# apache/brpc

Hardware: NVIDIA H100
Metric: echo QPS, 1 KB baidu_std (higher is better)
Workload: dtype u8

## Files before the change

brpc_b200/csrc/b2_api.cu:

```cuda
#include <cuda_runtime.h>
#include <dlfcn.h>
#include <stdio.h>
#include <time.h>
#include <stdlib.h>
#include <string.h>
#include <mutex>
#include <string>
#include <unordered_map>
#include <vector>
#include "b2_kernels.cuh"
#include "b2_h2.cuh"

using namespace b2;

static thread_local char g_err[512] = "";
static void set_err(const char* fmt, const char* a = "", const char* b = "") { snprintf(g_err, sizeof g_err, fmt, a, b); }

#define CU(call)                                                                          \
    do {                                                                                  \
        cudaError_t e_ = (call);                                                          \
        if (e_ != cudaSuccess) { set_err("%s: %s", #call, cudaGetErrorString(e_)); return B2_E_CUDA; } \
    } while (0)

namespace {
// ... 166 lines not shown
    ALLOC(c->d_slow_idx, sizeof(uint32_t) * (size_t)o->max_msgs);
    ALLOC(c->d_heads, (size_t)kHeadBytes * (size_t)o->max_msgs);
    ALLOC(c->d_slot, 4 * ((size_t)o->max_msgs + 1));
    ALLOC(c->d_scan_tmp, 4 * (size_t)scan_blocks);
    ALLOC(c->d_resp, (size_t)c->opt.max_resp_bytes + 1024);
    ALLOC(c->d_unz, 2 * (size_t)c->opt.max_resp_bytes + 1024);
    ALLOC(c->d_snappy_tab, (size_t)kSnappyWarps * kSnappyMaxTable * 2);
    ALLOC(c->d_hpack, sizeof(HpackState) * (size_t)B2_HPACK_MAX_CONNS);
    CU(cudaMemset(c->d_hpack, 0, sizeof(HpackState) * (size_t)B2_HPACK_MAX_CONNS));
    ALLOC(c->d_counters, 8 * B2_N_COUNTERS);
    ALLOC(c->d_totals, 64);
    ALLOC(c->d_methods, sizeof(DevMethod) * 64);
    ALLOC(c->d_crc_adv, (kCrcHotWords + kCrcTreeWords) * 4);
    ALLOC(c->d_meta, (size_t)o->max_runs * 28 + 16 * (size_t)c->max_tiles + 64);
    ALLOC(c->d_small, kSmallBlock);
    HALLOC(c->h_meta, (size_t)o->max_runs * 28 + 16 * (size_t)c->max_tiles + 64);
    HALLOC(c->h_small, kSmallBlock);
    HALLOC(c->h_run_status, sizeof(b2_run_status) * (size_t)o->max_runs);
    HALLOC(c->h_msgs, sizeof(b2_msg_desc) * (size_t)o->max_msgs);
    HALLOC(c->h_refs, sizeof(b2_resp_ref) * (size_t)o->max_msgs);
    HALLOC(c->h_resp, (size_t)c->opt.max_resp_bytes);
    HALLOC(c->h_totals, 64);
    HALLOC(c->h_run_tile_base, 4 * ((size_t)o->max_runs + 1));
    CU(cudaMemset(c->d_counters, 0, 8 * B2_N_COUNTERS));
    CU(cudaMemset(c->d_bytes, 0, (size_t)o->max_batch_bytes + 1024));
    CU(cudaStreamCreateWithFlags(&c->stream, cudaStreamNonBlocking));
    for (int i = 0; i <= kMaxStages; i++) CU(cudaEventCreate(&c->ev[i]));
    CU(cudaEventCreate(&c->ev_first)); CU(cudaEventCreate(&c->ev_last));
    crc_table_init();
    CU(cudaMemcpyToSymbol(c_crc_table, g_crc_tab_host, sizeof g_crc_tab_host));
    {
        std::vector<uint32_t> tab(kCrcHotWords + kCrcTreeWords);
        auto adv = [&](uint32_t x, int bytes) { for (int k = 0; k < bytes; k++) x = g_crc_tab_host[x & 0xff] ^ (x >> 8); return x; };
        for (int k = 0; k < 16; k++) for (uint32_t b = 0; b < 256; b++) tab[k * 256 + b] = adv(g_crc_tab_host[b], k);
        for (int j = 0; j < 4; j++) for (uint32_t b = 0; b < 256; b++) tab[(16 + j) * 256 + b] = adv(b << (8 * j), 512);
        for (int t = 0; t < 5; t++) for (int j = 0; j < 4; j++) for (uint32_t b = 0; b < 256; b++)
            tab[kCrcHotWords + (t * 4 + j) * 256 + b] = adv(b << (8 * j), 16 << t);
        CU(cudaMemcpy(c->d_crc_adv, tab.data(), tab.size() * 4, cudaMemcpyHostToDevice));
    }
    CU(cudaFuncSetAttribute(k_resolve, cudaFuncAttributeMaxDynamicSharedMemorySize, 200 * 1024));
    CU(cudaFuncSetAttribute(k_pack_slow<false>, cudaFuncAttributeMaxDynamicSharedMemorySize, (int)(8 * kSnapRing)));
    CU(cudaFuncSetAttribute(k_pack_tma<kPackGroup>, cudaFuncAttributeMaxDynamicSharedMemorySize, (int)(sizeof(PackWarpSmem) * kPackWarps)));
    CU(cudaFuncSetAttribute(k_pack_tma<kPackGroupSmall>, cudaFuncAttributeMaxDynamicSharedMemorySize, (int)(sizeof(PackWarpSmem) * kPackWarps)));
    if (const char* e = getenv("B2_PACK")) c->use_tma_pack = strcmp(e, "reg") != 0;
    if (const char* e = getenv("B2_SMALL")) c->use_fused_small = strcmp(e, "off") != 0;
    if (const char* e = getenv("B2_FUSED")) c->use_fused = strcmp(e, "off") != 0;
    CU(cudaFuncSetAttribute(k_fused, cudaFuncAttributeMaxDynamicSharedMemorySize, (int)(sizeof(FusedWarpSmem) * (kFusedWarps > kFusedWarpsDense ? kFusedWarps : kFusedWarpsDense))));
    CU(cudaFuncSetAttribute(k_small, cudaFuncAttributeMaxDynamicSharedMemorySize, (int)sizeof(SmallSmem)));
    *out = c;
    return B2_OK;
}

extern "C" int b2_set_server_identity(b2_ctx* c, const char* ip_port) {
    if (!c) return B2_E_INVAL;
    const size_t n = ip_port ? strlen(ip_port) : 0;
    if (n >= sizeof c->cfg.identity) { set_err("identity too long"); return B2_E_INVAL; }
    memset(c->cfg.identity, 0, sizeof c->cfg.identity);
    if (n) memcpy(c->cfg.identity, ip_port, n);
    c->cfg.identity_len = (uint32_t)n;
    return B2_OK;
}

extern "C" int b2_set_modes(b2_ctx* c, int input_mode, int resp_mode) {
    if (!c || (input_mode != B2_INPUT_COPY && input_mode != B2_INPUT_PULL) || (resp_mode != B2_RESP_COPY && resp_mode != B2_RESP_BY_REF && resp_mode != B2_RESP_IOVEC)) { set_err("bad mode"); return B2_E_INVAL; }
    static_assert(sizeof(b2_resp_ref) == sizeof(uint4), "b2_resp_ref is 16 bytes");
    static_assert(sizeof(b2_iovec) == sizeof(ulonglong2) && sizeof(void*) == 8, "b2_iovec is a 16-byte struct iovec");
    if (resp_mode == B2_RESP_IOVEC && !c->d_iov) {
        CU(cudaSetDevice(c->opt.device));
        if (cudaMalloc((void**)&c->d_iov, 32 * (size_t)c->opt.max_msgs) != cudaSuccess || cudaHostAlloc((void**)&c->h_iov, 32 * (size_t)c->opt.max_msgs, cudaHostAllocDefault) != cudaSuccess) {
            cudaFree(c->d_iov); c->d_iov = nullptr; cudaGetLastError(); set_err("allocation of the iovec list failed"); return B2_E_NOMEM;
        }
    }
    if (input_mode == B2_INPUT_PULL && !c->d_rows) {
        CU(cudaSetDevice(c->opt.device));
        const uint32_t tile = c->adaptive_tile ? 32768u : c->opt.tile_bytes;
        const size_t tiles = (size_t)c->opt.max_batch_bytes / tile + c->opt.max_runs + 1;
        const size_t rows = tiles * (tile >= 2048 ? kSpecKDense : kSpecK);
        if (cudaMalloc((void**)&c->d_rows, rows * 128) != cudaSuccess || cudaMalloc((void**)&c->d_frame_row, 4 * (size_t)c->opt.max_msgs) != cudaSuccess) {
            cudaFree(c->d_rows); c->d_rows = nullptr; cudaGetLastError(); set_err("cudaMalloc of the pull-mode row stash failed"); return B2_E_NOMEM;
        }
    }
    ring_halt(c);
    c->input_mode = input_mode; c->resp_mode = resp_mode; c->cfg.by_ref = resp_mode != B2_RESP_COPY; c->cfg.pull = input_mode == B2_INPUT_PULL; c->cfg.pull_vecs = resp_mode != B2_RESP_COPY ? 6u : 8u;
    c->uploaded = false; c->executed = false;
    return B2_OK;
}

extern "C" int b2_set_protocols(b2_ctx* c, uint32_t mask) {
    const uint32_t known = (1u << 1) | (1u << 2) | (1u << 3) | (1u << 4) | (1u << 12);
    if (!c || mask == 0 || (mask & ~known)) { set_err("unknown protocol in mask (baidu_std 1, streaming_rpc 2, hulu_pbrpc 3, sofa_pbrpc 4, nshead 12)"); return B2_E_INVAL; }
    ring_halt(c);
    c->cfg.proto_mask = mask;
    return B2_OK;
}

extern "C" int b2_set_stream_handler(b2_ctx* c, int kind) {
    if (!c || (kind != B2_STREAM_DESC_ONLY && kind != B2_STREAM_SNAPPY_UNCOMPRESS)) { set_err("bad stream handler"); return B2_E_INVAL; }
    c->cfg.stream_handler = (uint32_t)kind;
    return B2_OK;
}

extern "C" int b2_register_method(b2_ctx* c, const b2_method* m) {
    if (!c || !m || !m->service_full_name || !m->service_name || !m->method_name || !m->request_type_name) { set_err("null argument"); return B2_E_INVAL; }
    if (c->methods.size() >= 64) { set_err("method table full"); return B2_E_CAPACITY; }
    DevMethod d; memset(&d, 0, sizeof d);
    std::string full = std::string(m->service_full_name) + "." + m->method_name;
    if (full.size() >= sizeof d.full_method || strlen(m->service_name) >= sizeof d.service_short ||
        strlen(m->service_full_name) >= sizeof d.service_full || strlen(m->request_type_name) >= sizeof d.request_type) {
        set_err("method names too long"); return B2_E_INVAL;
    }
    memcpy(d.full_method, full.data(), full.size()); d.full_method_len = (uint32_t)full.size();
    d.service_short_len = (uint32_t)strlen(m->service_name); memcpy(d.service_short, m->service_name, d.service_short_len);
    d.service_full_len = (uint32_t)strlen(m->service_full_name); memcpy(d.service_full, m->service_full_name, d.service_full_len);
    d.request_type_len = (uint32_t)strlen(m->request_type_name); memcpy(d.request_type, m->request_type_name, d.request_type_len);
    d.handler = m->handler; d.echo_attachment = m->echo_attachment;
    d.response_checksum_type = m->response_checksum_type; d.response_compress_type = m->response_compress_type;
    ring_halt(c);
    c->methods.push_back(d);
    c->cfg.n_methods = (uint32_t)c->methods.size();
    CU(cudaSetDevice(c->opt.device));
    CU(cudaMemcpy(c->d_methods, c->methods.data(), sizeof(DevMethod) * c->methods.size(), cudaMemcpyHostToDevice));
    return (int)c->methods.size() - 1;
}

static BatchPtrs make_ptrs(b2_ctx* c) {
    BatchPtrs B;
    B.bytes = c->d_bytes; B.runs = c->d_runs; B.run_tile_base = c->d_run_tile_base; B.tiles = c->d_tiles;
    B.tile_base = c->d_tile_base; B.tile_scratch = c->d_tile_scratch; B.tile_spec = c->d_tile_spec; B.run_status = c->d_run_status; B.frame_off = c->d_frame_off; B.frame_run = c->d_frame_run; B.frame_row = c->d_frame_row; B.rows = c->d_rows; B.msgs = c->d_msgs;
    B.aux = c->d_aux; B.jobs = c->d_jobs; B.refs = c->d_refs; B.slow_idx = c->d_slow_idx; B.heads = c->d_heads; B.slot = c->d_slot; B.scan_tmp = c->d_scan_tmp; B.resp = c->d_resp; B.unz = c->d_unz; B.snappy_tab = c->d_snappy_tab; B.counters = c->d_counters;
    B.totals = c->d_totals; B.methods = c->d_methods; B.crc_adv = c->d_crc_adv;
    B.n_runs = c->n_runs; B.n_tiles = c->n_tiles; B.max_msgs = c->opt.max_msgs; B.max_resp = c->opt.max_resp_bytes;
    B.runs = reinterpret_cast<const b2_run*>(c->d_meta);
    B.run_tile_base = reinterpret_cast<const uint32_t*>(c->d_meta + (size_t)c->n_runs * sizeof(b2_run));
    B.tile_info = reinterpret_cast<const uint4*>(c->d_meta + c->meta_tile_off);
    if (c->input_mode == B2_INPUT_PULL) B.bytes = c->pull_bytes;
    if (c->small) {
        B.refs = reinterpret_cast<uint4*>(c->d_small + c->small_off_refs);
        B.totals = reinterpret_cast<uint32_t*>(c->d_small);
        B.run_status = reinterpret_cast<b2_run_status*>(c->d_small + c->small_off_rs);
        B.msgs = reinterpret_cast<b2_msg_desc*>(c->d_small + c->small_off_msgs);
        B.resp = c->d_small + c->small_off_resp;
        B.max_msgs = c->small_msgs; B.max_resp = c->small_resp;
    }
    return B;
}

extern "C" int b2_batch_upload(b2_ctx* c, const void* bytes, uint32_t nbytes, const b2_run* runs, uint32_t n_runs) {
    if (!c || (!bytes && nbytes) || (!runs && n_runs)) { set_err("null argument"); return B2_E_INVAL; }
    if ((c->input_mode != B2_INPUT_PULL && nbytes > c->opt.max_batch_bytes) || nbytes >= (1u << 31) || n_runs > c->opt.max_runs) { set_err("batch exceeds ctx capacity"); return B2_E_CAPACITY; }
    uint64_t covered = 0; for (uint32_t r = 0; r < n_runs; r++) covered += runs[r].length;
    if (c->input_mode == B2_INPUT_PULL && covered > c->opt.max_batch_bytes) { set_err("runs exceed ctx capacity"); return B2_E_CAPACITY; }
    c->covered = covered;
    CU(cudaSetDevice(c->opt.device));
    if (c->adaptive_tile) {
        uint32_t t = 8192;
        const uint32_t per_tile = c->input_mode == B2_INPUT_PULL ? 48u : 6u;
        if (c->input_mode == B2_INPUT_PULL && t < 32768) t = 32768;
        while (t < (1u << 20) && t < per_tile * c->avg_frame) t <<= 1;
        c->cfg.tile_bytes = t; c->cfg.tile_shift = 0; while ((1u << c->cfg.tile_shift) < t) c->cfg.tile_shift++;
    }
    const uint32_t shift = c->cfg.tile_shift, tile = c->cfg.tile_bytes;
    c->dense = tile >= 2048 && c->avg_frame && (uint64_t)c->avg_frame * kSpecK < tile;
    c->cfg.spec_k = c->dense ? kSpecKDense : kSpecK;
    uint64_t nt = 0; uint32_t max_rt = 0;
    for (uint32_t r = 0; r < n_runs; r++) {
        if ((runs[r].offset & 15u) || (uint64_t)runs[r].offset + runs[r].length > nbytes) { set_err("run offset must be 16-aligned and inside the batch"); return B2_E_INVAL; }
        c->h_run_tile_base[r] = (uint32_t)nt;
        const uint32_t t = (uint32_t)(((uint64_t)runs[r].length + tile - 1) >> shift);
        nt += t; if (t > max_rt) max_rt = t;
    }
    c->h_run_tile_base[n_runs] = (uint32_t)nt;
    if (nt > c->max_tiles) { set_err("too many tiles"); return B2_E_CAPACITY; }
    c->n_runs = n_runs; c->n_tiles = (uint32_t)nt; c->nbytes = nbytes; c->max_run_tiles = max_rt; c->host_bytes = bytes;
    const size_t tile_off = ((size_t)n_runs * sizeof(b2_run) + 4 * ((size_t)n_runs + 1) + 15) & ~(size_t)15;
    const size_t meta_bytes = tile_off + 16 * (size_t)nt;
    c->meta_tile_off = tile_off;
    if (n_runs) memcpy(c->h_meta, runs, (size_t)n_runs * sizeof(b2_run));
    memcpy(c->h_meta + (size_t)n_runs * sizeof(b2_run), c->h_run_tile_base, 4 * ((size_t)n_runs + 1));
    {
        uint32_t* ti = reinterpret_cast<uint32_t*>(c->h_meta + tile_off);
        for (uint32_t r = 0; r < n_runs; r++) {
            const uint32_t t0 = c->h_run_tile_base[r], t1 = c->h_run_tile_base[r + 1];
            for (uint32_t t = t0; t < t1; t++) { uint32_t* q = ti + 4 * (size_t)t; q[0] = runs[r].offset; q[1] = runs[r].length; q[2] = t - t0; q[3] = r | (runs[r].flags << 24); }
        }
    }
    c->h2_last_in = 0; c->h2_last_out = 0;
    if (c->input_mode == B2_INPUT_PULL) {
        void* dp = nullptr;
        if (nbytes && cudaHostGetDevicePointer(&dp, const_cast<void*>(bytes), 0) != cudaSuccess) {
            cudaGetLastError(); set_err("B2_INPUT_PULL: bytes must be pinned + mapped memory from b2_block_alloc"); return B2_E_INVAL;
        }
        c->pull_bytes = static_cast<const uint8_t*>(dp);
    } else if (nbytes) CU(cudaMemcpyAsync(c->d_bytes, bytes, nbytes, cudaMemcpyHostToDevice, c->stream));
    CU(cudaMemcpyAsync(c->d_meta, c->h_meta, meta_bytes, cudaMemcpyHostToDevice, c->stream));
    c->small = c->allow_small && nbytes <= kSmallBytes && n_runs <= kSmallRuns && n_runs > 0;
    if (c->small) {
        uint32_t mb = nbytes / 12 + 1; if (mb > kSmallMsgs) mb = kSmallMsgs;
        if (mb > c->opt.max_msgs) mb = c->opt.max_msgs;
        c->small_msgs = mb; c->small_resp = nbytes + mb * 80 + 2048;
        c->small_off_rs = 64; c->small_off_msgs = 64 + n_runs * 32; c->small_off_refs = c->small_off_msgs + mb * 64;
        c->small_off_resp = (c->small_off_refs + mb * 16 + 255u) & ~255u;
        c->small_total = c->small_off_resp + c->small_resp;
    }
    if (const char* e = getenv("B2_STAGE_MASK")) c->stage_mask = (uint32_t)atoi(e);
    c->uploaded = true; c->executed = false;
    return B2_OK;
}

static int launch_pipeline(b2_ctx* c) {
    const BatchPtrs B = make_ptrs(c);
    DevConfig C = c->cfg;
    const bool fused = c->use_fused && !c->slow_heavy && !c->small && c->input_mode == B2_INPUT_COPY && c->resp_mode == B2_RESP_COPY && c->use_tma_pack &&
                       (((uint64_t)c->nbytes + 255) & ~255ull) + 4096 <= c->opt.max_resp_bytes;
    C.fused = fused ? 1u : 0u; C.ovf_base = (c->nbytes + 255u) & ~255u; c->fused_last = fused;
    cudaStream_t s = c->stream;
    int st = 0; uint32_t launches = 0;
    const bool prof = c->profile_stages;
    auto mark = [&](const char* name) { if (prof) { c->stage_names[st] = name; cudaEventRecord(c->ev[st + 1], s); st++; } };
    const uint32_t mask = c->stage_mask;
    if (mask & 1) CU(cudaMemsetAsync(B.totals, 0, 48, s));
    CU(cudaEventRecord(c->ev[0], s));
    if (c->n_runs == 0) { c->n_stages = 0; c->last_launches = 0; return B2_OK; }
    if (c->small && c->use_fused_small && !prof) {
        k_small<<<1, kSmallThreads, sizeof(SmallSmem), s>>>(B, C);
        c->stage_names[0] = "fused_small"; cudaEventRecord(c->ev[1], s);
        c->n_stages = 1; c->last_launches = 1;
        CU(cudaGetLastError());
        return B2_OK;
    }
    const uint32_t sms = c->n_sms;
    if (mask & 1) {
    if (c->n_tiles) {
        k_tile_search<<<(c->n_tiles * 32 + 255) / 256, 256, 0, s>>>(B, C); launches++; mark("tile_search");
        if (C.pull) k_tile_walk_pull<<<(uint32_t)(((uint64_t)c->n_tiles * 8 + 127) / 128), 128, 0, s>>>(B, C);
        else k_tile_walk<<<(c->n_tiles + 127) / 128, 128, 0, s>>>(B, C);
        launches++; mark("tile_walk");
    }
    {
        size_t smem = (size_t)c->max_run_tiles * 12;
        if (smem > 200 * 1024) smem = 0;
        k_resolve<<<c->n_runs, 256, smem, s>>>(B, C, smem == 0 ? 1u : 0u); launches++; mark("resolve");
    }
    if (fused) {
        const uint32_t fw = c->avg_frame && !c->dense ? kFusedWarps : kFusedWarpsDense;
        if (c->n_tiles) { k_fused<<<sms, fw * 32, sizeof(FusedWarpSmem) * fw, s>>>(B, C); launches++; mark("fused"); }
    } else {
    if (c->n_tiles) { k_frame_table<<<(uint32_t)(((uint64_t)c->n_tiles * C.spec_k + 255) / 256), 256, 0, s>>>(B, C); launches++; mark("frame_table"); }
    k_decode<<<sms * B2_DECODE_MIN_BLOCKS, kDecodeWarps * 32, 0, s>>>(B, C); launches++; mark("decode");
    k_scan_blocks<<<sms, kScanBlock, 0, s>>>(B); launches++;
    mark("scan");
    }
    }
    if (fused) {
        if (mask & 4) { k_pack_slow<true><<<sms * B2_SLOW_MIN_BLOCKS, 256, 0, s>>>(B, C); launches++; mark("pack_slow"); }
    } else if (c->use_tma_pack) {
        if (mask & 4) {
            if (c->slow_heavy || c->cfg.by_ref) { C.verify_done = 1; k_crc_verify<<<sms * 6, 256, 0, s>>>(B, C); launches++; mark("crc_verify"); }
            k_pack_slow<false><<<sms * B2_SLOW_MIN_BLOCKS, 256, 8 * kSnapRing, s>>>(B, C); launches++; mark("pack_slow");
        }
        if (mask & 2) {
            if ((c->avg_frame && c->avg_frame < 640) || c->cfg.by_ref) k_pack_tma<kPackGroupSmall><<<sms, kPackWarps * 32, sizeof(PackWarpSmem) * kPackWarps, s>>>(B, C);
            else k_pack_tma<kPackGroup><<<sms, kPackWarps * 32, sizeof(PackWarpSmem) * kPackWarps, s>>>(B, C);
            launches++; mark("pack");
        }
    } else { k_pack<<<sms * B2_PACK_MIN_BLOCKS, 256, 0, s>>>(B, C); launches++; mark("pack"); }
    if (c->resp_mode == B2_RESP_IOVEC && !c->small) {
        k_emit_iov<<<sms * 4, 256, 0, s>>>(B, c->d_iov, (unsigned long long)(uintptr_t)c->h_resp, (unsigned long long)(uintptr_t)c->host_bytes);
        launches++; mark("emit_iov");
    }
    if (!prof) { c->stage_names[0] = "pipeline"; cudaEventRecord(c->ev[1], s); st = 1; }
    c->n_stages = st; c->last_launches = launches;
    CU(cudaGetLastError());
    return B2_OK;
}

extern "C" int b2_batch_execute(b2_ctx* c, float* kernel_ms, uint32_t* n_launches) {
    if (!c || !c->uploaded) { set_err("no batch uploaded"); return B2_E_INVAL; }
    CU(cudaSetDevice(c->opt.device));
    c->profile_stages = true;
    int rc = launch_pipeline(c);
    c->profile_stages = false;
    if (rc != B2_OK) return rc;
    CU(cudaStreamSynchronize(c->stream));
    float ms = 0.f;
    if (c->n_stages) CU(cudaEventElapsedTime(&ms, c->ev[0], c->ev[c->n_stages]));
    c->last_kernel_ms = ms; c->executed = true;
    if (kernel_ms) *kernel_ms = ms;
    if (n_launches) *n_launches = c->last_launches;
    return B2_OK;
}

extern "C" int b2_batch_execute_many(b2_ctx* c, uint32_t steps, float* total_ms, uint32_t* n_launches) {
    if (!c || !c->uploaded || steps == 0) { set_err("no batch uploaded"); return B2_E_INVAL; }
    CU(cudaSetDevice(c->opt.device));
    cudaEvent_t e0, e1;
    CU(cudaEventCreate(&e0)); CU(cudaEventCreate(&e1));
    CU(cudaEventRecord(e0, c->stream));
    uint32_t launches = 0;
    for (uint32_t i = 0; i < steps; i++) {
        int rc = launch_pipeline(c);
        if (rc != B2_OK) return rc;
        launches += c->last_launches;
    }
    CU(cudaEventRecord(e1, c->stream));
    CU(cudaStreamSynchronize(c->stream));
    float ms = 0.f;
    CU(cudaEventElapsedTime(&ms, e0, e1));
    cudaEventDestroy(e0); cudaEventDestroy(e1);
    c->executed = true;
    if (c->n_stages) { float t = 0.f; cudaEventElapsedTime(&t, c->ev[0], c->ev[c->n_stages]); c->last_kernel_ms = t; }
    if (total_ms) *total_ms = ms;
    if (n_launches) *n_launches = launches;
    return B2_OK;
}

extern "C" int b2_batch_launch(b2_ctx* c) {
    if (!c || !c->uploaded) { set_err("no batch uploaded"); return B2_E_INVAL; }
    CU(cudaSetDevice(c->opt.device));
    if (c->first_pending) { CU(cudaEventRecord(c->ev_first, c->stream)); c->first_pending = false; }
    int rc = launch_pipeline(c);
    if (rc != B2_OK) return rc;
    CU(cudaEventRecord(c->ev_last, c->stream));
    c->executed = true;
    return B2_OK;
}
extern "C" int b2_batch_wait(b2_ctx* c) {
    if (!c) return B2_E_INVAL;
    CU(cudaSetDevice(c->opt.device));
    CU(cudaStreamSynchronize(c->stream));
    c->first_pending = true;
    return B2_OK;
}
extern "C" int b2_elapsed_ms(b2_ctx* a, b2_ctx* b, float* ms) {
    if (!a || !b || !ms) return B2_E_INVAL;
    CU(cudaSetDevice(a->opt.device));
    CU(cudaEventElapsedTime(ms, a->ev_first, b->ev_last));
    return B2_OK;
}

static void refs_to_iov(b2_ctx* c, b2_batch_result* out, const void* host_bytes) {
    b2_run_status* rs = const_cast<b2_run_status*>(out->runs);
    for (uint32_t r = 0; r < out->n_runs; r++) rs[r].n_unanswered = 0;
    for (uint32_t i = 0; i < out->n_msgs; i++) {
        const b2_msg_desc& d = out->msgs[i];
        b2_iovec a = { const_cast<uint8_t*>(out->resp), 0 }, b = a;
        if (d.status == B2_MSG_ECHOED || d.status == B2_MSG_ERROR_REPLIED) {
            const b2_resp_ref rf = d.status == B2_MSG_ECHOED ? out->refs[i] : b2_resp_ref{0, 0, 0, 0};
            a.iov_base = const_cast<uint8_t*>(out->resp) + d.resp_off; a.iov_len = rf.src_len ? rf.prefix_len : d.resp_len;
            if (rf.src_len) { b.iov_base = const_cast<uint8_t*>(static_cast<const uint8_t*>(host_bytes)) + rf.src_off; b.iov_len = rf.src_len; }
        } else rs[d.run_idx].n_unanswered++;
        c->h_iov[2 * (size_t)i] = a; c->h_iov[2 * (size_t)i + 1] = b;
    }
    out->iov = c->h_iov; out->refs = nullptr;
}

static int download_normal(b2_ctx* c, b2_batch_result* out) {
    CU(cudaMemcpyAsync(c->h_totals, c->d_totals, 48, cudaMemcpyDeviceToHost, c->stream));
    CU(cudaStreamSynchronize(c->stream));
    if (c->n_runs && c->fused_last) {
        const bool heavy = (uint64_t)c->h_totals[3] * 8 > c->h_totals[0];
        if ((c->h_totals[2] & 2u) && !(c->h_totals[2] & 1u)) {
            c->slow_heavy = true;
            int rc = launch_pipeline(c); if (rc != B2_OK) return rc;
            CU(cudaMemcpyAsync(c->h_totals, c->d_totals, 48, cudaMemcpyDeviceToHost, c->stream));
            CU(cudaStreamSynchronize(c->stream));
        }
        c->slow_heavy = heavy || c->slow_heavy;
    } else if (c->n_runs && c->slow_heavy && !c->small) {
        c->slow_heavy = ((uint64_t)c->h_totals[3] + c->h_totals[7]) * 8 > c->h_totals[0];
    }
    if (c->n_runs && (c->h_totals[2] & 3u)) {
        set_err(c->h_totals[2] & 1u ? "more messages than max_msgs" : "responses exceed max_resp_bytes"); return B2_E_CAPACITY;
    }
    if (c->n_runs && c->fused_last) c->h_totals[1] = ((c->nbytes + 255u) & ~255u) + c->h_totals[9];
    const uint32_t n_msgs = c->n_runs ? c->h_totals[0] : 0, resp_bytes = c->n_runs ? c->h_totals[1] : 0;
    if (c->n_runs) CU(cudaMemcpyAsync(c->h_run_status, c->d_run_status, sizeof(b2_run_status) * c->n_runs, cudaMemcpyDeviceToHost, c->stream));
    if (n_msgs) CU(cudaMemcpyAsync(c->h_msgs, c->d_msgs, sizeof(b2_msg_desc) * (size_t)n_msgs, cudaMemcpyDeviceToHost, c->stream));
    if (resp_bytes) CU(cudaMemcpyAsync(c->h_resp, c->d_resp, resp_bytes, cudaMemcpyDeviceToHost, c->stream));
    const bool iovec = c->resp_mode == B2_RESP_IOVEC;
    if (n_msgs && c->cfg.by_ref && !iovec) CU(cudaMemcpyAsync(c->h_refs, c->d_refs, sizeof(b2_resp_ref) * (size_t)n_msgs, cudaMemcpyDeviceToHost, c->stream));
    if (n_msgs && iovec) CU(cudaMemcpyAsync(c->h_iov, c->d_iov, 32 * (size_t)n_msgs, cudaMemcpyDeviceToHost, c->stream));
    CU(cudaStreamSynchronize(c->stream));
    out->refs = c->cfg.by_ref && !iovec ? c->h_refs : nullptr;
    out->iov = iovec ? c->h_iov : nullptr;
    out->runs = c->h_run_status; out->n_runs = c->n_runs;
    out->msgs = c->h_msgs; out->n_msgs = n_msgs;
    out->resp = c->h_resp; out->resp_bytes = resp_bytes;
    return B2_OK;
}

extern "C" int b2_batch_download(b2_ctx* c, b2_batch_result* out) {
    if (!c || !out || !c->executed) { set_err("no executed batch"); return B2_E_INVAL; }
    CU(cudaSetDevice(c->opt.device));
    memset(out, 0, sizeof *out);
    if (c->small) {
        if (!c->small_copy_queued) CU(cudaMemcpyAsync(c->h_small, c->d_small, c->small_total, cudaMemcpyDeviceToHost, c->stream));
        c->small_copy_queued = false;
        CU(cudaStreamSynchronize(c->stream));
        const uint32_t* tot = reinterpret_cast<const uint32_t*>(c->h_small);
        if (tot[2] & 3u) {
            c->small = false;
            int rc = launch_pipeline(c);
            if (rc != B2_OK) return rc;
            rc = download_normal(c, out);
            if (rc != B2_OK) return rc;
        } else {
            out->runs = reinterpret_cast<const b2_run_status*>(c->h_small + c->small_off_rs); out->n_runs = c->n_runs;
// ... 798 lines not shown
```

brpc_b200/csrc/b2_kernels.cuh:

```cuda
#pragma once
#include <cuda_runtime.h>
#include "b2_core.cuh"
#include "b2_inflate.cuh"

namespace b2 {

enum TileKind : uint8_t { kRanOff = 0, kStop = 1, kAmbig = 2 };

struct __align__(16) TileRec {
    uint32_t entry;
    uint32_t exit;
    uint32_t count;
    uint8_t kind;
    int8_t last_proto;
    uint8_t live;
    int8_t pf_in;
};

struct __align__(16) MsgAux {
    uint32_t msg_off;
    uint32_t msg_len;
    uint32_t att_len;
    uint32_t att_off;
    uint32_t cks_off;
    uint32_t cks_len;
    uint32_t svc_off, svc_len;
    uint32_t mth_off, mth_len;
    uint32_t pad;
    uint32_t err_kind;
};
struct __align__(16) PackJob {
    uint32_t src_off;
    uint32_t bulk_len;
    uint16_t head_len;
    uint8_t pad;
    uint8_t fast;
    uint32_t slot_len;
};
constexpr uint32_t kHeadBytes = 96;

enum ErrKind : uint32_t { kErrNone = 0, kErrAttachment, kErrNoService, kErrNoMethod, kErrParseRequest };

struct DevMethod {
    char full_method[200];
    uint32_t full_method_len;
    char service_short[64];  uint32_t service_short_len;
    char service_full[120];  uint32_t service_full_len;
    char request_type[96];   uint32_t request_type_len;
    int32_t handler, echo_attachment, response_checksum_type, response_compress_type;
};
struct DevConfig {
    uint64_t max_body_size;
    uint32_t tile_bytes, tile_shift;
    uint32_t n_methods;
    uint32_t identity_len;
    uint32_t stream_handler;
    uint32_t spec_k;
    uint32_t by_ref;
    uint32_t verify_done;
    uint32_t proto_mask;
    uint32_t fused;
    uint32_t ovf_base;
    uint32_t pull_vecs;
    uint32_t pull;
    char identity[64];
};

struct BatchPtrs {
    const uint8_t* bytes;
    const b2_run* runs;
    const uint32_t* run_tile_base;
    const uint4* tile_info;
    TileRec* tiles;
    uint32_t* tile_base;
    uint32_t* tile_scratch;
    uint32_t* tile_spec;
    b2_run_status* run_status;
    uint32_t* frame_off;
    uint32_t* frame_run;
    uint32_t* frame_row;
    uint4* rows;
    b2_msg_desc* msgs;
    MsgAux* aux;
    PackJob* jobs;
    uint4* refs;
    uint32_t* slow_idx;
    uint8_t* heads;
    uint32_t* slot;
    uint32_t* scan_tmp;
    uint8_t* resp;
    uint8_t* unz;
    uint16_t* snappy_tab;
    unsigned long long* counters;
    uint32_t* totals;
    const DevMethod* methods;
    const uint32_t* crc_adv;
    uint32_t n_runs, n_tiles, max_msgs, max_resp;
};

template <bool kSpec, typename Emit>
B2_HD void walk_tile(const uint8_t* run, uint32_t len, uint32_t entry, int pf_in, uint32_t tile_end,
                     uint64_t max_body, bool client, TileRec& t, Emit emit, uint32_t mask = kProtoMaskDefault) {
    uint32_t pos = entry, count = 0;
    int pf = kSpec ? -1 : pf_in, last = 0;
    uint8_t kind = kRanOff;
    while (pos < tile_end) {
        const Step s = cut_input_message(run, len, pos, pf, max_body, client, mask);
        if (kSpec && count == 0 && (s.popped || (s.index != 12 && nshead_claims(run, len, pos, max_body, mask)))) { kind = kAmbig; break; }
        if (s.err != B2_PARSE_OK) { kind = kStop; break; }
        emit(count, s);
        count++; last = s.index; pf = s.index; pos = s.new_pos;
    }
    t.entry = entry; t.exit = pos; t.count = count; t.kind = kind; t.last_proto = (int8_t)last;
}
struct NoEmit { B2_HD void operator()(uint32_t, const Step&) const {} };
constexpr uint32_t kSpecK = 16;
constexpr uint32_t kSpecKDense = 128;
constexpr uint8_t kKindRewalked = 0x80;
struct EmitSpec {
    uint32_t* out; uint32_t run_off, cap;
    __device__ __forceinline__ void operator()(uint32_t i, const Step& s) const {
        if (i < cap) out[i] = (run_off + s.frame_pos) | ((uint32_t)(s.index != 1) << 31);
    }
};

#if defined(__CUDACC__)

__device__ __forceinline__ uint32_t find_run(const uint32_t* base, uint32_t n_runs, uint32_t tile) {
    uint32_t lo = 0, hi = n_runs;
    while (hi - lo > 1) { const uint32_t mid = (lo + hi) >> 1; if (__ldg(base + mid) <= tile) lo = mid; else hi = mid; }
    return lo;
}
__device__ __forceinline__ bool is_magic(uint32_t w) { return w == kMagicPRPC || w == kMagicSTRM; }
#ifndef B2_SEARCH_FIRST
#define B2_SEARCH_FIRST 2
#endif

__global__ void __launch_bounds__(256, 6) k_tile_search(BatchPtrs B, DevConfig C) {
    const uint32_t warp = (blockIdx.x * blockDim.x + threadIdx.x) >> 5, lane = threadIdx.x & 31;
    if (warp >= B.n_tiles) return;
    const uint4 ti = __ldg(B.tile_info + warp);
    const uint32_t k = ti.z;
    const uint8_t* base = B.bytes + ti.x;
    const uint32_t len = ti.y;
    uint32_t entry = kNone;
    if (k == 0) {
        entry = 0;
    } else {
        const uint32_t t0 = k << C.tile_shift;
        const uint32_t t1 = min(t0 + C.tile_bytes, len);
        for (uint32_t c0 = t0; c0 < t1 && entry == kNone; c0 += (c0 == t0 ? 512u * B2_SEARCH_FIRST : 2048u)) {
            const int nwin = c0 == t0 ? B2_SEARCH_FIRST : 4;
            uint4 v[4]; uint32_t nx[4];
            #pragma unroll
            for (int u = 0; u < 4; u++) {
                const uint32_t p0 = c0 + u * 512 + lane * 16;
                v[u] = make_uint4(0, 0, 0, 0); nx[u] = 0;
                if (u < nwin && p0 < t1) {
                    v[u] = __ldg(reinterpret_cast<const uint4*>(base + p0));
                    nx[u] = __ldg(reinterpret_cast<const uint32_t*>(base + p0 + 16));
                }
            }
            #pragma unroll
            for (int u = 0; u < 4; u++) {
                if (entry != kNone || u >= nwin) break;
                const uint32_t w0 = c0 + u * 512, p0 = w0 + lane * 16;
                const uint32_t w[5] = { v[u].x, v[u].y, v[u].z, v[u].w, nx[u] };
                uint32_t mask = 0, mkind = 0;
                const bool ext = (C.proto_mask & ((1u << 3) | (1u << 4))) != 0;
                #pragma unroll
                for (int k4 = 0; k4 < 4; k4++) {
                    uint32_t e = __vcmpeq4(w[k4], 0x50505050u) | __vcmpeq4(w[k4], 0x53535353u);
                    if (ext) e |= __vcmpeq4(w[k4], 0x48484848u);
                    while (e) {
                        const int b = (__ffs(e) - 1) >> 3;
                        e &= ~(0xffu << (8 * b));
                        const int j = 4 * k4 + b;
                        const uint32_t word = __funnelshift_r(w[k4], w[k4 + 1], b * 8);
                        const bool other = ext && ((word == kMagicHULU && (C.proto_mask & 8u)) || (word == kMagicSOFA && (C.proto_mask & 16u)));
                        if ((is_magic(word) || other) && p0 + j + 4 <= len && p0 + j < t1) { mask |= 1u << j; if (other) mkind |= (word == kMagicHULU ? 1u : 2u) << (2 * j); }
                    }
                }
                uint32_t any = __ballot_sync(0xffffffffu, mask != 0);
                const uint32_t n5 = __shfl_down_sync(0xffffffffu, v[u].y, 1), n6 = __shfl_down_sync(0xffffffffu, v[u].z, 1);
                while (any && entry == kNone) {
                    const int src = __ffs(any) - 1;
                    uint32_t m = __shfl_sync(0xffffffffu, mask, src);
                    const uint32_t kinds = __shfl_sync(0xffffffffu, mkind, src);
                    while (m && entry == kNone) {
                        const int jj = __ffs(m) - 1;
                        const uint32_t p = w0 + src * 16 + jj;
                        m &= m - 1;
                        const uint32_t kind = (kinds >> (2 * jj)) & 3u;
                        if (kind == 2) { entry = p; break; }
                        uint32_t body_le = 0, meta_le = 0;
                        if (src < 31) {
                            const uint32_t q = (uint32_t)(jj + 4) >> 2, sh = ((uint32_t)(jj + 4) & 3u) * 8u;
                            const uint32_t a1 = w[1], a2 = w[2], a3 = w[3], a4 = w[4];
                            const uint32_t x0 = q == 1 ? a1 : q == 2 ? a2 : q == 3 ? a3 : a4;
                            const uint32_t x1 = q == 1 ? a2 : q == 2 ? a3 : q == 3 ? a4 : n5;
                            const uint32_t x2 = q == 1 ? a3 : q == 2 ? a4 : q == 3 ? n5 : n6;
                            body_le = __shfl_sync(0xffffffffu, __funnelshift_r(x0, x1, sh), src);
                            meta_le = __shfl_sync(0xffffffffu, __funnelshift_r(x1, x2, sh), src);
                        } else if (p + 12 <= len) {
                            body_le = load_le32(base + p + 4); meta_le = load_le32(base + p + 8);
                        } else continue;
                        const uint32_t body = kind == 1 ? body_le : __byte_perm(body_le, 0, 0x0123), meta = kind == 1 ? meta_le : __byte_perm(meta_le, 0, 0x0123);
                        if (meta <= body && (uint64_t)body <= C.max_body_size) entry = p;
                    }
                    any &= any - 1;
                }
            }
        }
    }
    if (lane == 0) B.tiles[warp].entry = entry;
}

struct HdrWords { uint32_t w0, w1, w2, w3; };
__device__ __forceinline__ HdrWords load_hdr_words(const uint8_t* p) {
    const uint32_t* q = reinterpret_cast<const uint32_t*>((uintptr_t)p & ~(uintptr_t)3);
    HdrWords h; h.w0 = __ldg(q); h.w1 = __ldg(q + 1); h.w2 = __ldg(q + 2); h.w3 = __ldg(q + 3);
    return h;
}
template <typename Emit>
__device__ __forceinline__ void walk_tile_spec(const uint8_t* run, uint32_t len, uint32_t entry, uint32_t tile_end,
                                               uint64_t max_body, bool client, TileRec& t, Emit emit, uint32_t mask) {
    uint32_t pos = entry, count = 0, prev_len = 0, pre_pos = kNone;
    int pf = -1, last = 0;
    uint8_t kind = kRanOff;
    HdrWords pre; pre.w0 = pre.w1 = pre.w2 = pre.w3 = 0;
    while (pos < tile_end) {
        Step s;
        bool fast = false;
        if (len - pos >= 12) {
            const HdrWords h = pre_pos == pos ? pre : load_hdr_words(run + pos);
            const uint32_t guess = pos + prev_len;
            if (prev_len && guess < tile_end && (uint64_t)guess + 12 <= len) { pre = load_hdr_words(run + guess); pre_pos = guess; }
            else pre_pos = kNone;
            const uint32_t sh = 8u * (pos & 3u);
            const uint32_t h0 = sh ? __funnelshift_r(h.w0, h.w1, sh) : h.w0, h1 = sh ? __funnelshift_r(h.w1, h.w2, sh) : h.w1,
                           h2 = sh ? __funnelshift_r(h.w2, h.w3, sh) : h.w2;
            const int idx = h0 == kMagicPRPC ? 1 : h0 == kMagicSTRM ? 2 : 0;
            const uint32_t body = __byte_perm(h1, 0, 0x0123), meta = __byte_perm(h2, 0, 0x0123);
            if (idx && ((mask >> idx) & 1u) && pf != 12 && (uint64_t)body <= max_body && (uint64_t)(len - pos) >= 12ull + body && meta <= body) {
                s.err = B2_PARSE_OK; s.index = idx; s.pf = idx; s.frame_pos = pos; s.new_pos = pos + 12 + body; s.body = body; s.meta = meta; s.popped = false;
                fast = true;
            }
        }
        if (!fast) s = cut_input_message(run, len, pos, pf, max_body, client, mask);
        if (count == 0 && (s.popped || (s.index != 12 && nshead_claims(run, len, pos, max_body, mask)))) { kind = kAmbig; break; }
        if (s.err != B2_PARSE_OK) { kind = kStop; break; }
        emit(count, s);
        count++; last = s.index; pf = s.index; prev_len = s.new_pos - pos; pos = s.new_pos;
    }
    t.entry = entry; t.exit = pos; t.count = count; t.kind = kind; t.last_proto = (int8_t)last;
}

__global__ void __launch_bounds__(128) k_tile_walk(BatchPtrs B, DevConfig C) {
    const uint32_t t = blockIdx.x * blockDim.x + threadIdx.x;
    if (t >= B.n_tiles) return;
    const uint4 ti = __ldg(B.tile_info + t);
    const uint32_t k = ti.z;
    b2_run run; run.offset = ti.x; run.length = ti.y; run.flags = ti.w >> 24;
    TileRec rec;
    rec.entry = B.tiles[t].entry; rec.exit = 0; rec.count = 0; rec.kind = kStop; rec.last_proto = 0; rec.live = 0; rec.pf_in = -1;
    if (rec.entry != kNone) {
        EmitSpec e; e.out = B.tile_spec + (size_t)t * C.spec_k; e.run_off = run.offset; e.cap = C.spec_k;
        walk_tile_spec(B.bytes + run.offset, run.length, rec.entry, (k + 1) << C.tile_shift, C.max_body_size, (run.flags & B2_RUN_CLIENT) != 0, rec, e, run_mask(C.proto_mask, run.flags));
    }
    B.tiles[t] = rec;
}

__global__ void __launch_bounds__(128) k_tile_walk_pull(BatchPtrs B, DevConfig C) {
    const uint32_t g = blockIdx.x * blockDim.x + threadIdx.x;
    const uint32_t t = g >> 3, sub = threadIdx.x & 7u, lane = threadIdx.x & 31u;
    if (t >= B.n_tiles) return;
    const uint32_t gmask = 0xffu << (lane & 24u), l0 = lane & 24u;
    const uint4 ti = __ldg(B.tile_info + t);
    const uint32_t k = ti.z, len = ti.y;
    const uint8_t* run = B.bytes + ti.x;
    const bool client = ((ti.w >> 24) & B2_RUN_CLIENT) != 0;
    const uint32_t pmask = run_mask(C.proto_mask, ti.w >> 24);
    const uint32_t tile_end = (k + 1) << C.tile_shift, cap = C.spec_k;
    uint32_t* spec = B.tile_spec + (size_t)t * cap;
    uint4* rows = B.rows + (size_t)t * cap * 8;
    TileRec rec;
    rec.entry = B.tiles[t].entry; rec.exit = 0; rec.count = 0; rec.kind = kStop; rec.last_proto = 0; rec.live = 0; rec.pf_in = -1;
    if (rec.entry != kNone) {
        uint32_t pos = rec.entry, count = 0; int pf = -1, last = 0; uint8_t kind = kRanOff;
        while (pos < tile_end) {
            bool fast = false; uint32_t new_pos = pos, frame_pos = pos; int idx = 0, err = B2_PARSE_OK; bool popped = false;
            uint4 v = make_uint4(0, 0, 0, 0);
            if (len - pos >= 12) {
                if (sub < C.pull_vecs) v = __ldg(reinterpret_cast<const uint4*>(run + (pos & ~15u)) + sub);
                const uint32_t a0 = __shfl_sync(gmask, v.x, l0), a1 = __shfl_sync(gmask, v.y, l0), a2 = __shfl_sync(gmask, v.z, l0), a3 = __shfl_sync(gmask, v.w, l0);
                const uint32_t b0 = __shfl_sync(gmask, v.x, l0 + 1), b1 = __shfl_sync(gmask, v.y, l0 + 1), b2 = __shfl_sync(gmask, v.z, l0 + 1);
                const uint32_t q = (pos & 15u) >> 2, sh = 8u * (pos & 3u);
                const uint32_t w0 = q == 0 ? a0 : q == 1 ? a1 : q == 2 ? a2 : a3, w1 = q == 0 ? a1 : q == 1 ? a2 : q == 2 ? a3 : b0;
                const uint32_t w2 = q == 0 ? a2 : q == 1 ? a3 : q == 2 ? b0 : b1, w3 = q == 0 ? a3 : q == 1 ? b0 : q == 2 ? b1 : b2;
                const uint32_t h0 = sh ? __funnelshift_r(w0, w1, sh) : w0, h1 = sh ? __funnelshift_r(w1, w2, sh) : w1, h2 = sh ? __funnelshift_r(w2, w3, sh) : w2;
                idx = h0 == kMagicPRPC ? 1 : h0 == kMagicSTRM ? 2 : 0;
                const uint32_t body = __byte_perm(h1, 0, 0x0123), meta = __byte_perm(h2, 0, 0x0123);
                if (idx && ((pmask >> idx) & 1u) && pf != 12 && (uint64_t)body <= C.max_body_size && (uint64_t)(len - pos) >= 12ull + body && meta <= body) { fast = true; new_pos = pos + 12 + body; }
            }
            if (count == 0 && ((pmask >> 12) & 1u)) {
                int amb = 0;
                if (sub == 0) amb = nshead_claims(run, len, pos, C.max_body_size, pmask) ? 1 : 0;
                if (__shfl_sync(gmask, amb, l0)) { kind = kAmbig; break; }
            }
            if (!fast) {
                Step s; s.err = 0; s.index = 0; s.new_pos = 0; s.frame_pos = 0; s.popped = false;
                if (sub == 0) s = cut_input_message(run, len, pos, pf, C.max_body_size, client, pmask);
                err = __shfl_sync(gmask, s.err, l0); idx = __shfl_sync(gmask, s.index, l0); new_pos = __shfl_sync(gmask, s.new_pos, l0);
                frame_pos = __shfl_sync(gmask, s.frame_pos, l0); popped = __shfl_sync(gmask, (int)s.popped, l0) != 0;
                if (count == 0 && popped) { kind = kAmbig; break; }
                if (err != B2_PARSE_OK) { kind = kStop; break; }
                if (sub < C.pull_vecs) v = __ldg(reinterpret_cast<const uint4*>(run + (frame_pos & ~15u)) + sub);
            }
            if (count < cap) {
                if (sub == 0) spec[count] = (ti.x + frame_pos) | ((uint32_t)(idx != 1) << 31);
                if (sub < C.pull_vecs) rows[(size_t)count * 8 + sub] = v;
            }
            count++; last = idx; pf = idx; pos = new_pos;
        }
        rec.exit = pos; rec.count = count; rec.kind = kind; rec.last_proto = (int8_t)last;
    }
    if (sub == 0) B.tiles[t] = rec;
}

__device__ __forceinline__ void run_prefix_body(const BatchPtrs& B, uint32_t* s_warp, uint32_t* s_carry) {
    const uint32_t lane = threadIdx.x & 31, wid = threadIdx.x >> 5, nw = blockDim.x >> 5;
    if (threadIdx.x == 0) *s_carry = 0;
    __syncthreads();
    for (uint32_t base = 0; base < B.n_runs; base += blockDim.x) {
        const uint32_t i = base + threadIdx.x;
        uint32_t v = i < B.n_runs ? __ldcg(&B.run_status[i].n_msgs) : 0, x = v;
        #pragma unroll
        for (int d = 1; d < 32; d <<= 1) { const uint32_t y = __shfl_up_sync(0xffffffffu, x, d); if (lane >= (uint32_t)d) x += y; }
        if (lane == 31) s_warp[wid] = x;
        __syncthreads();
        uint32_t wbase = 0, wtot = 0;
        for (uint32_t w = 0; w < nw; w++) { const uint32_t t = s_warp[w]; if (w < wid) wbase += t; wtot += t; }
        const uint32_t carry = *s_carry;
        if (i < B.n_runs) B.run_status[i].first_msg = carry + wbase + x - v;
        __syncthreads();
        if (threadIdx.x == 0) *s_carry = carry + wtot;
        __syncthreads();
    }
    if (threadIdx.x == 0) { B.totals[0] = *s_carry; if (*s_carry > B.max_msgs) B.totals[2] |= 1u; }
}

constexpr uint32_t kLinkOk = 0x80000000u;
constexpr uint32_t kLinkStop = 0x40000000u;
constexpr uint32_t kLinkEnd = 0x20000000u;
constexpr uint32_t kLinkBroken = 0x10000000u;
constexpr uint32_t kLinkRewalk = 0x08000000u;

__device__ __forceinline__ uint32_t make_link(const TileRec& t, const TileRec* tiles, uint32_t nt, uint32_t shift) {
    if (t.entry == kNone || t.kind == kAmbig) return kLinkRewalk;
    if (t.kind == kStop) return kLinkStop;
    const uint32_t j = t.exit >> shift;
    if (j >= nt) return kLinkEnd;
    return (tiles[j].entry == t.exit ? kLinkOk : kLinkBroken) | j;
}

__global__ void __launch_bounds__(256) k_resolve(BatchPtrs B, DevConfig C, uint32_t use_scratch) {
    extern __shared__ uint32_t sm[];
    const uint32_t r = blockIdx.x;
    const b2_run run = B.runs[r];
    const uint8_t* base = B.bytes + run.offset;
    const uint32_t len = run.length;
    const uint32_t tb = B.run_tile_base[r], nt = B.run_tile_base[r + 1] - tb;
    TileRec* tiles = B.tiles + tb;
    const bool fits = !use_scratch;
    uint32_t* link = fits ? sm : B.tile_scratch + 3ull * tb;
    uint32_t* cp = link + nt;
    uint32_t* live = cp + nt;
    __shared__ uint32_t s_final_pos, s_warp_sum[8], s_warp_pf[8], s_carry_sum, s_carry_pf;
    const uint32_t rmask = run_mask(C.proto_mask, run.flags);
    const bool pf_decides = (run.flags & B2_RUN_CLIENT) && !(rmask & kProtoMaskDump) && (rmask & ~((1u << B2_PROTOCOL_BAIDU_STD) | (1u << B2_PROTOCOL_STREAMING_RPC))) != 0;
    for (uint32_t k = threadIdx.x; k < nt; k += blockDim.x) {
        const TileRec t = tiles[k];
        link[k] = ((k == 0 && t.entry != 0) || pf_decides) ? kLinkRewalk : make_link(t, tiles, nt, C.tile_shift);
        cp[k] = (t.count << 4) | ((uint32_t)t.last_proto & 15u);
        live[k] = 0;
    }
    __shared__ uint32_t s_first_bad;
    if (threadIdx.x == 0) s_first_bad = nt ? nt - 1 : 0;
    __syncthreads();
    {
        uint32_t mine = nt;
        for (uint32_t k = threadIdx.x; k + 1 < nt; k += blockDim.x)
            if (link[k] != (kLinkOk | (k + 1))) { mine = k; break; }
        if (mine < nt) atomicMin(&s_first_bad, mine);
    }
    __syncthreads();
    const uint32_t first_bad = s_first_bad;
    for (uint32_t k = threadIdx.x; k < first_bad; k += blockDim.x) live[k] = 1;
    __syncthreads();
    if (threadIdx.x == 0) {
        uint32_t k = first_bad, pos = 0;
        bool via_ok = first_bad > 0;
        while (k < nt) {
            uint32_t v = link[k];
            if (v & kLinkRewalk) {
                if (via_ok) pos = tiles[k].entry;
                int pf = run.preferred_proto;
                for (uint32_t j = k; j-- > 0;) if (live[j] && (cp[j] >> 4)) { pf = (int)(cp[j] & 15u); break; }
                TileRec t; t.live = 0; t.pf_in = 0;
                walk_tile<false>(base, len, pos, pf, (k + 1) << C.tile_shift, C.max_body_size, (run.flags & B2_RUN_CLIENT) != 0, t, NoEmit(), run_mask(C.proto_mask, run.flags));
                tiles[k].entry = t.entry; tiles[k].exit = t.exit; tiles[k].count = t.count; tiles[k].kind = t.kind | kKindRewalked; tiles[k].last_proto = t.last_proto;
                cp[k] = (t.count << 4) | ((uint32_t)t.last_proto & 15u);
                v = make_link(t, tiles, nt, C.tile_shift);
                link[k] = v;
            }
            live[k] = 1;
            if (v & kLinkOk) { k = v & 0x07ffffffu; via_ok = true; continue; }
            if (v & kLinkBroken) {
                const uint32_t j = v & 0x07ffffffu;
                pos = tiles[k].exit; k = j; link[j] = kLinkRewalk; via_ok = false;
                continue;
            }
            pos = tiles[k].exit;
// ... 2120 lines not shown
```

Before: 1.020 billion.

## Fuse tile search and walk into persistent speculative-stride front kernel

For non-pull input, tile entry search and the tile walk are merged into one persistent kernel, k_tile_front, which takes work chunks through an atomic counter. Each 8-lane group walks its tile speculatively at a predicted frame stride and validates several candidate headers in parallel. It falls back to the serial parser when the guess fails, and issues L2 prefetches for the search region. The change also seeds avg_frame on the host from the first frame header of each run, and relaunches pack_slow with twice the blocks at 128 threads each. The goal is fewer launches and less serial per-frame walking, at the cost of more divergence and complexity. It also depends on a counter slot (totals+10) that is zeroed by the existing memset.

Measured after the change: 1.094 billion (median of 6 runs). +7.2%, better.

```diff
diff --git a/brpc_b200/csrc/b2_api.cu b/brpc_b200/csrc/b2_api.cu
--- a/brpc_b200/csrc/b2_api.cu
+++ b/brpc_b200/csrc/b2_api.cu
@@ -342,6 +342,16 @@
     if (c->input_mode == B2_INPUT_PULL && covered > c->opt.max_batch_bytes) { set_err("runs exceed ctx capacity"); return B2_E_CAPACITY; }
     c->covered = covered;
     CU(cudaSetDevice(c->opt.device));
+    if (!c->avg_frame && n_runs) {
+        uint64_t sum = 0; uint32_t n = 0;
+        for (uint32_t r = 0; r < n_runs; r++) {
+            if (runs[r].length < 12 || (uint64_t)runs[r].offset + 12 > nbytes) continue;
+            const uint8_t* p = static_cast<const uint8_t*>(bytes) + runs[r].offset;
+            const uint32_t magic = load_le32(p), body = load_be32(p + 4);
+            if ((magic == kMagicPRPC || magic == kMagicSTRM) && body <= c->cfg.max_body_size) { sum += 12ull + body; n++; }
+        }
+        if (n) c->avg_frame = (uint32_t)(sum / n);
+    }
     if (c->adaptive_tile) {
         uint32_t t = 8192;
         const uint32_t per_tile = c->input_mode == B2_INPUT_PULL ? 48u : 6u;
@@ -420,11 +430,12 @@
     }
     const uint32_t sms = c->n_sms;
     if (mask & 1) {
-    if (c->n_tiles) {
+    if (c->n_tiles && C.pull) {
         k_tile_search<<<(c->n_tiles * 32 + 255) / 256, 256, 0, s>>>(B, C); launches++; mark("tile_search");
-        if (C.pull) k_tile_walk_pull<<<(uint32_t)(((uint64_t)c->n_tiles * 8 + 127) / 128), 128, 0, s>>>(B, C);
-        else k_tile_walk<<<(c->n_tiles + 127) / 128, 128, 0, s>>>(B, C);
-        launches++; mark("tile_walk");
+        k_tile_walk_pull<<<(uint32_t)(((uint64_t)c->n_tiles * 8 + 127) / 128), 128, 0, s>>>(B, C); launches++; mark("tile_walk");
+    } else if (c->n_tiles) {
+        const uint32_t chunks = (c->n_tiles + 8 * kFrontChunk - 1) / (8 * kFrontChunk), grid = chunks < sms * 4 ? chunks : sms * 4;
+        k_tile_front<<<grid, 256, 0, s>>>(B, C); launches++; mark("tile_front");
     }
     {
         size_t smem = (size_t)c->max_run_tiles * 12;
@@ -442,7 +453,7 @@
     }
     }
     if (fused) {
-        if (mask & 4) { k_pack_slow<true><<<sms * B2_SLOW_MIN_BLOCKS, 256, 0, s>>>(B, C); launches++; mark("pack_slow"); }
+        if (mask & 4) { k_pack_slow<true><<<sms * B2_SLOW_MIN_BLOCKS * 2, 128, 0, s>>>(B, C); launches++; mark("pack_slow"); }
     } else if (c->use_tma_pack) {
         if (mask & 4) {
             if (c->slow_heavy || c->cfg.by_ref) { C.verify_done = 1; k_crc_verify<<<sms * 6, 256, 0, s>>>(B, C); launches++; mark("crc_verify"); }
diff --git a/brpc_b200/csrc/b2_kernels.cuh b/brpc_b200/csrc/b2_kernels.cuh
--- a/brpc_b200/csrc/b2_kernels.cuh
+++ b/brpc_b200/csrc/b2_kernels.cuh
@@ -136,14 +136,10 @@
 #define B2_SEARCH_FIRST 2
 #endif
 
-__global__ void __launch_bounds__(256, 6) k_tile_search(BatchPtrs B, DevConfig C) {
-    const uint32_t warp = (blockIdx.x * blockDim.x + threadIdx.x) >> 5, lane = threadIdx.x & 31;
-    if (warp >= B.n_tiles) return;
-    const uint4 ti = __ldg(B.tile_info + warp);
-    const uint32_t k = ti.z;
-    const uint8_t* base = B.bytes + ti.x;
-    const uint32_t len = ti.y;
+__device__ __forceinline__ uint32_t search_tile_entry(const uint8_t* base, uint32_t len, uint32_t k, uint32_t lane, const DevConfig& C,
+                                                      uint32_t& first_len) {
     uint32_t entry = kNone;
+    first_len = 0;
     if (k == 0) {
         entry = 0;
     } else {
@@ -206,13 +202,22 @@
                             body_le = load_le32(base + p + 4); meta_le = load_le32(base + p + 8);
                         } else continue;
                         const uint32_t body = kind == 1 ? body_le : __byte_perm(body_le, 0, 0x0123), meta = kind == 1 ? meta_le : __byte_perm(meta_le, 0, 0x0123);
-                        if (meta <= body && (uint64_t)body <= C.max_body_size) entry = p;
+                        if (meta <= body && (uint64_t)body <= C.max_body_size) { entry = p; first_len = 12u + body; }
                     }
                     any &= any - 1;
                 }
             }
         }
     }
+    return entry;
+}
+
+__global__ void __launch_bounds__(256, 6) k_tile_search(BatchPtrs B, DevConfig C) {
+    const uint32_t warp = (blockIdx.x * blockDim.x + threadIdx.x) >> 5, lane = threadIdx.x & 31;
+    if (warp >= B.n_tiles) return;
+    const uint4 ti = __ldg(B.tile_info + warp);
+    uint32_t first_len;
+    const uint32_t entry = search_tile_entry(B.bytes + ti.x, ti.y, ti.z, lane, C, first_len);
     if (lane == 0) B.tiles[warp].entry = entry;
 }
 
@@ -269,6 +274,88 @@
         walk_tile_spec(B.bytes + run.offset, run.length, rec.entry, (k + 1) << C.tile_shift, C.max_body_size, (run.flags & B2_RUN_CLIENT) != 0, rec, e, run_mask(C.proto_mask, run.flags));
     }
     B.tiles[t] = rec;
+}
+
+constexpr uint32_t kFrontLanes = 8;
+template <typename Emit>
+__device__ __forceinline__ void walk_tile_group(const uint8_t* run, uint32_t len, uint32_t entry, uint32_t stride, uint32_t tile_end,
+                                                uint64_t max_body, bool client, TileRec& t, Emit emit, uint32_t mask, uint32_t lane) {
+    const uint32_t j = lane % kFrontLanes, base = lane - j;
+    uint32_t pos = entry, count = 0;
+    int pf = -1, last = 0;
+    uint8_t kind = kRanOff;
+    bool live = entry != kNone && pos < tile_end;
+    while (__ballot_sync(0xffffffffu, live)) {
+        const uint64_t pj = (uint64_t)pos + (uint64_t)j * stride;
+        bool ok = false;
+        int idx = 0;
+        uint32_t next = 0;
+        if (live && (j == 0 || stride != 0) && pj < tile_end && pj + 12 <= len) {
+            const HdrWords h = load_hdr_words(run + pj);
+            const uint32_t sh = 8u * ((uint32_t)pj & 3u);
+            const uint32_t h0 = sh ? __funnelshift_r(h.w0, h.w1, sh) : h.w0, h1 = sh ? __funnelshift_r(h.w1, h.w2, sh) : h.w1,
+                           h2 = sh ? __funnelshift_r(h.w2, h.w3, sh) : h.w2;
+            idx = h0 == kMagicPRPC ? 1 : h0 == kMagicSTRM ? 2 : 0;
+            const uint32_t body = __byte_perm(h1, 0, 0x0123), meta = __byte_perm(h2, 0, 0x0123);
+            ok = idx && ((mask >> idx) & 1u) && (j != 0 || pf != 12) && (uint64_t)body <= max_body && (uint64_t)(len - (uint32_t)pj) >= 12ull + body && meta <= body;
+            next = (uint32_t)pj + 12u + body;
+        }
+        const uint32_t prev_next = __shfl_sync(0xffffffffu, next, j ? lane - 1 : lane);
+        const uint32_t bad = ~(__ballot_sync(0xffffffffu, ok && (j == 0 || prev_next == (uint32_t)pj)) >> base) & ((1u << kFrontLanes) - 1u);
+        const uint32_t n = bad ? (uint32_t)__ffs(bad) - 1u : kFrontLanes;
+        const uint32_t src = base + (n ? n - 1 : 0);
+        const uint32_t at = __shfl_sync(0xffffffffu, (uint32_t)pj, src), at_next = __shfl_sync(0xffffffffu, next, src);
+        const int at_idx = __shfl_sync(0xffffffffu, idx, src);
+        if (!live) continue;
+        if (n) {
+            if (count == 0 && nshead_claims(run, len, pos, max_body, mask)) { kind = kAmbig; live = false; continue; }
+            if (j < n) { Step s; s.err = B2_PARSE_OK; s.index = idx; s.pf = idx; s.frame_pos = (uint32_t)pj; s.new_pos = next; s.body = 0; s.meta = 0; s.popped = false; emit(count + j, s); }
+            pos = at_next; pf = last = at_idx; stride = at_next - at; count += n;
+        } else {
+            const Step s = cut_input_message(run, len, pos, pf, max_body, client, mask);
+            if (count == 0 && (s.popped || (s.index != 12 && nshead_claims(run, len, pos, max_body, mask)))) { kind = kAmbig; live = false; continue; }
+            if (s.err != B2_PARSE_OK) { kind = kStop; live = false; continue; }
+            if (j == 0) emit(count, s);
+            count++; last = s.index; pf = s.index; stride = s.new_pos - pos; pos = s.new_pos;
+        }
+        live = pos < tile_end;
+    }
+    t.entry = entry; t.exit = pos; t.count = count; t.kind = kind; t.last_proto = (int8_t)last;
+}
+
+__device__ __forceinline__ void prefetch_l2_line(const void* p) { asm volatile("prefetch.global.L2 [%0];" ::"l"(p)); }
+constexpr uint32_t kFrontChunk = 32 / kFrontLanes;
+__global__ void __launch_bounds__(256, 4) k_tile_front(BatchPtrs B, DevConfig C) {
+    const uint32_t lane = threadIdx.x & 31, g = lane / kFrontLanes;
+    for (;;) {
+        uint32_t t0 = 0;
+        if (lane == 0) t0 = atomicAdd(B.totals + 10, kFrontChunk);
+        t0 = __shfl_sync(0xffffffffu, t0, 0);
+        if (t0 >= B.n_tiles) return;
+        const uint32_t t = t0 + g;
+        uint4 ti = make_uint4(0, 0, 0, 0);
+        if (t < B.n_tiles) {
+            ti = __ldg(B.tile_info + t);
+            const uint32_t at = (ti.z << C.tile_shift) + (lane % kFrontLanes) * 128u;
+            if ((lane % kFrontLanes) * 128u < 512u * B2_SEARCH_FIRST && at < ti.y) prefetch_l2_line(B.bytes + ti.x + at);
+        }
+        uint32_t entry = kNone, stride = 0;
+        for (uint32_t i = 0; i < kFrontChunk && t0 + i < B.n_tiles; i++) {
+            const uint32_t src = i * kFrontLanes;
+            uint32_t s_i;
+            const uint32_t e_i = search_tile_entry(B.bytes + __shfl_sync(0xffffffffu, ti.x, src), __shfl_sync(0xffffffffu, ti.y, src),
+                                                   __shfl_sync(0xffffffffu, ti.z, src), lane, C, s_i);
+            if (g == i) { entry = e_i; stride = s_i; }
+        }
+        TileRec rec;
+        EmitSpec e; e.out = B.tile_spec + (size_t)t * C.spec_k; e.run_off = ti.x; e.cap = C.spec_k;
+        const uint32_t flags = ti.w >> 24;
+        walk_tile_group(B.bytes + ti.x, ti.y, entry, stride, (ti.z + 1) << C.tile_shift, C.max_body_size, (flags & B2_RUN_CLIENT) != 0, rec, e,
+                        run_mask(C.proto_mask, flags), lane);
+        if (entry == kNone) { rec.exit = 0; rec.count = 0; rec.kind = kStop; rec.last_proto = 0; }
+        rec.live = 0; rec.pf_in = -1;
+        if (lane % kFrontLanes == 0 && t < B.n_tiles) B.tiles[t] = rec;
+    }
 }
 
 __global__ void __launch_bounds__(128) k_tile_walk_pull(BatchPtrs B, DevConfig C) {
```
